# JuliaPhylo/PhyloGaussianBeliefProp.jl

Measured on AMD Instinct MI355X. Metric: clique-tree messages/sec (calibrate!: postorder+preorder), 16-trait BM, higher is better.
Workload: dtype f64; 1 GPU; cfg3: homogeneous BM, 16 traits, 50000-tip random bifurcating tree (seed 3), cliquetree, fixed root; clusters=99998, sepsets=99997, tree_depth=38, parallelism=single GPU

## Files before the change

### include/pgbp.h

```cpp
#ifndef PGBP_H
#define PGBP_H

#include <stdint.h>

#ifdef __cplusplus
extern "C" {
#endif

#define PGBP_VERSION 1
#define PGBP_MAX_DIM 384

enum pgbp_status {
  PGBP_OK = 0,
  PGBP_ERR_INVALID = 1,
  PGBP_ERR_HIP = 2,
  PGBP_ERR_NOT_TREE = 3,
  PGBP_ERR_TOO_LARGE = 4,
  PGBP_ERR_NO_DEVICE = 5,
  PGBP_ERR_STATE = 6
};

typedef struct pgbp_desc {
  int32_t n_clusters;
  int32_t n_sepsets;
// ... 35 lines not shown
                            const int32_t* pa_j, const int32_t* ch_j);
int64_t pgbp_plan_packed_size(const pgbp_plan* p);
int64_t pgbp_plan_residual_size(const pgbp_plan* p);
int32_t pgbp_plan_n_messages(const pgbp_plan* p);
int  pgbp_plan_traversal_sizes(const pgbp_plan* p, int32_t tree, int32_t dir,
                               int32_t* n_levels, int32_t* n_tasks, int32_t* n_entries);
int  pgbp_plan_traversal(const pgbp_plan* p, int32_t tree, int32_t dir, int32_t* level_off,
                         int32_t* task_off, int32_t* entry_msg, int32_t* entry_edge, int32_t* entry_reuse);
int  pgbp_plan_level_nfast(const pgbp_plan* p, int32_t tree, int32_t dir, int32_t* level_nfast);
int  pgbp_plan_groups(const pgbp_plan* p, int32_t tree, int32_t dir, int32_t* level_ngroups, int32_t* tail_levels,
                      int32_t* records, int32_t* tail_records);
int  pgbp_plan_chunks(const pgbp_plan* p, int32_t tree, int32_t dir, int32_t* n_chunks, int32_t* info, int32_t* wg_off,
                      int32_t* records);
int  pgbp_plan_prologues(const pgbp_plan* p, int32_t tree, int32_t dir, int32_t* level_pro, int32_t* tail_pro,
                         int32_t* chunk_pro);
int  pgbp_plan_chains(const pgbp_plan* p, int32_t tree, int32_t dir, int32_t* tail_chain, int32_t* chunk_chain);
int  pgbp_plan_records(const pgbp_plan* p, int32_t tree, int32_t dir, int32_t* n_records, int32_t* level_first,
                       int32_t* task_first, uint8_t* records);
int  pgbp_plan_rows(const pgbp_plan* p, int32_t tree, int32_t dir, int64_t* n_rows, int64_t* level_row0,
                    int32_t* level_nrows, int32_t* rowmap);
int  pgbp_plan_onschedule(const pgbp_plan* p, int32_t* n_levels, int32_t* cluster_level, int32_t* msg_level,
                          int32_t* walk_pos);
const char* pgbp_plan_last_error(const pgbp_plan* p);

int  pgbp_create(const pgbp_desc* desc, pgbp_engine** out);
void pgbp_destroy(pgbp_engine* e);
const char* pgbp_last_error(const pgbp_engine* e);
int64_t pgbp_packed_size(const pgbp_engine* e);
int64_t pgbp_residual_size(const pgbp_engine* e);
int32_t pgbp_n_messages(const pgbp_engine* e);
// ... 249 lines not shown
```

### phylogaussianbeliefprop.jl_amd/_lib.py

```python
import ctypes as C
import os

import numpy as np

os.environ.setdefault("HIP_FORCE_DEV_KERNARG", "1")

_HERE = os.path.dirname(os.path.abspath(__file__))
LIB_PATH = os.environ.get("PGBP_LIB", os.path.join(_HERE, "csrc", "libpgbp.so"))

PGBP_OK, ERR_INVALID, ERR_HIP, ERR_NOT_TREE, ERR_TOO_LARGE, ERR_NO_DEVICE, ERR_STATE = range(7)
PGBP_MAX_DIM = 384


class PgbpError(RuntimeError):
    def __init__(self, code, msg):
        super().__init__(f"pgbp error {code}: {msg}")
        self.code = code
        self.msg = msg


class Desc(C.Structure):
    _fields_ = [("n_clusters", C.c_int32), ("n_sepsets", C.c_int32),
                ("dims", C.POINTER(C.c_int32)), ("sepset_clusters", C.POINTER(C.c_int32)),
                ("scope_off", C.POINTER(C.c_int64)), ("scope_idx", C.POINTER(C.c_int32)),
# ... 38 lines not shown
_I64P = C.POINTER(C.c_int64)
_F64P = C.POINTER(C.c_double)
SYMBOLS = {
    "pgbp_plan_create": (C.c_int, [C.POINTER(Desc), C.POINTER(_P)]),
    "pgbp_plan_destroy": (None, [_P]),
    "pgbp_plan_set_schedule": (C.c_int, [_P, C.c_int32, _I32P, _I32P, _I32P]),
    "pgbp_plan_packed_size": (C.c_int64, [_P]),
    "pgbp_plan_residual_size": (C.c_int64, [_P]),
    "pgbp_plan_n_messages": (C.c_int32, [_P]),
    "pgbp_plan_traversal_sizes": (C.c_int, [_P, C.c_int32, C.c_int32, _I32P, _I32P, _I32P]),
    "pgbp_plan_traversal": (C.c_int, [_P, C.c_int32, C.c_int32, _I32P, _I32P, _I32P, _I32P, _I32P]),
    "pgbp_plan_level_nfast": (C.c_int, [_P, C.c_int32, C.c_int32, _I32P]),
    "pgbp_plan_groups": (C.c_int, [_P, C.c_int32, C.c_int32, _I32P, _I32P, _I32P, _I32P]),
    "pgbp_plan_chunks": (C.c_int, [_P, C.c_int32, C.c_int32, _I32P, _I32P, _I32P, _I32P]),
    "pgbp_plan_prologues": (C.c_int, [_P, C.c_int32, C.c_int32, _I32P, _I32P, _I32P]),
    "pgbp_plan_chains": (C.c_int, [_P, C.c_int32, C.c_int32, _I32P, _I32P]),
    "pgbp_plan_records": (C.c_int, [_P, C.c_int32, C.c_int32, _I32P, _I32P, _I32P, C.c_void_p]),
    "pgbp_plan_rows": (C.c_int, [_P, C.c_int32, C.c_int32, C.POINTER(C.c_int64), C.POINTER(C.c_int64), _I32P, _I32P]),
    "pgbp_plan_onschedule": (C.c_int, [_P, _I32P, _I32P, _I32P, _I32P]),
    "pgbp_residual_threshold": (C.c_double, [C.c_double, C.c_double]),
    "pgbp_plan_last_error": (C.c_char_p, [_P]),
    "pgbp_create": (C.c_int, [C.POINTER(Desc), C.POINTER(_P)]),
    "pgbp_destroy": (None, [_P]),
    "pgbp_last_error": (C.c_char_p, [_P]),
    "pgbp_packed_size": (C.c_int64, [_P]),
    "pgbp_residual_size": (C.c_int64, [_P]),
    "pgbp_n_messages": (C.c_int32, [_P]),
    "pgbp_belief_dim": (C.c_int32, [_P, C.c_int32]),
    "pgbp_set_beliefs": (C.c_int, [_P, _F64P, C.c_int32]),
    "pgbp_get_beliefs": (C.c_int, [_P, _F64P]),
# ... 192 lines not shown
```

### phylogaussianbeliefprop.jl_amd/csrc/pgbp_engine.hip

```cpp
#include <hip/hip_runtime.h>

#include <algorithm>
#include <climits>
#include <limits>
#include <cmath>
#include <cstdlib>
#include <cstdio>
#include <cstring>
#include <iterator>
#include <memory>
#include <string>
#include <vector>

#include "pgbp_devmem.hpp"
#include "pgbp_internal.hpp"
#include "pgbp_kernels.hpp"
#include "pgbp_lgmodel.hpp"
#include "pgbp_sites_host.hpp"
#include "pgbp_topology.hpp"

using namespace pgbp;

namespace {

// ... 209 lines not shown
  S.n_msgs = e->plan.n_msgs();
  S.update_resnorm = o ? o->update_residualnorm : 1;
  S.atol = o ? o->atol : 1e-5;
  S.thr = e->d_thr.get();
  S.logtab = reinterpret_cast<const double2*>(e->d_logtab.get());
  const int sp = e->plan.fast_p > 0 ? e->plan.fast_p : 0;
  S.thr_h_p = e->h_thr.empty() ? 0.0 : e->h_thr[sp];
  S.thr_J_p = e->h_thr.empty() ? 0.0 : e->h_thr[PGBP_MAX_DIM + 1 + sp];
  S.bs16 = e->layout_bs16 ? 1 : 0;
  S.fast_p = e->plan.fast_p;
  S.sm = e->layout_sm ? 1 : 0;
  S.n_sites = e->plan.n_sites;
  S.packed_off = e->d_packed_off.get();
  S.rpacked_off = e->d_rpacked_off.get();
  S.sep_zero = 0;
  S.notcal = nullptr;
  if (e->layout_sm) {
    S.pool = e->sm.pool.get();
    S.rpool = e->sm.rpool.get();
  }
  return S;
}

__global__ __launch_bounds__(256) void clear_poison_if_failed(const unsigned long long* __restrict__ fail, int n_sites,
                                                              int32_t* __restrict__ poison, int64_t n_words) {
  __shared__ int any;
  if (threadIdx.x == 0) any = 0;
  __syncthreads();
  for (int s = threadIdx.x; s < n_sites; s += blockDim.x)
    if (is_failure_key(fail[s])) any = 1;
// ... 205 lines not shown
      const int e0 = tr.task_off[t0], e1 = tr.task_off[t0 + nt];
      int level_s = 0;
      for (int q = e0; q < e1; ++q) level_s = std::max(level_s, (int)e->plan.msgs[tr.entries[q].msg].s);
      const auto b0 = std::lower_bound(d.kl_big.begin(), d.kl_big.end(), e0), b1 = std::lower_bound(d.kl_big.begin(), d.kl_big.end(), e1);
      const int n_big = (int)(b1 - b0);
      e->kl_flags_clean = e->kl_div_clean = false;
      if (n_big == 0 || ensure_ws(e, (int64_t)n_big * e->plan.n_sites * kldiv_ws_doubles(level_s)) == PGBP_OK)
        launch_residual_kldiv(S, d.d_entries.get(), e0, e1 - e0, level_s, e->d_kldiv.get(), e->d_klflags.get(), e->plan.n_sites, stop_below, e->st,
                              d.d_kl_big.get() + (b0 - d.kl_big.begin()), n_big, e->d_ws.get());
      else
        e->enqueue_rc = PGBP_ERR_HIP;
    }
  }
}

void enqueue_tree(pgbp_engine* e, const DevState& S, int tree, int dirs, unsigned long long pair_index, bool kl = false,
                  int* n_launches = nullptr) {
  const Tree& T = e->plan.trees[tree];
  const unsigned long long seq_base = pair_index * seq_stride(e);
  const unsigned long long stop_post = seq_base, stop_pre = seq_base + (unsigned long long)T.pa.size();
  const int np = (dirs & 1) ? tail_levels(e, T.post, kl) : 0, nq = (dirs & 2) ? tail_levels(e, T.pre, kl) : 0;
  const int nlev_post = (int)T.post.level_off.size() - 1, nlev_pre = (int)T.pre.level_off.size() - 1;
  if (dirs & 1) enqueue_levels(e, S, T.post, e->dpost[tree], 0, nlev_post - np, seq_base, stop_post, kl, n_launches);
  if (np + nq > 0) {
    const size_t first = (size_t)(np > 0 ? 0 : T.post.tail_levels) * kTailWaves;
    launch_loop_or_tail(e, S, e->d_tail[tree].get() + first, e->d_tail_pros[tree] ? e->d_tail_pros[tree].get() + first : nullptr, np + nq,
                        np, seq_base, stop_post, stop_pre, nullptr, 0);
    if (n_launches) *n_launches += 1;
  }
  if (dirs & 2) enqueue_levels(e, S, T.pre, e->dpre[tree], nq, nlev_pre, seq_base, stop_pre, kl, n_launches);
}

void enqueue_pair_and_iscal(pgbp_engine* e, const DevState& S, int tree, unsigned long long pair, bool kl, int32_t* d_out,
                            int* n_launches = nullptr) {
  const Plan& p = e->plan;
  const bool fused = e->layout_sm && !kl && S.update_resnorm != 0 && (int)p.trees[tree].pa.size() == p.n_sepsets;
  if (fused) {
    (void)hipMemsetAsync(e->d_notcal.get(), 0, sizeof(int32_t) * (size_t)p.n_sites, e->st);
    DevState S1 = S;
    S1.notcal = e->d_notcal.get();
    enqueue_tree(e, S1, tree, 3, pair, kl, n_launches);
    launch_iscal_from_notcal(e->d_notcal.get(), d_out, p.n_sites, e->st);
  } else {
    enqueue_tree(e, S, tree, 3, pair, kl, n_launches);
    launch_reduce_flags(e->d_flags.get(), p.n_msgs(), p.n_sites, d_out, e->st, e->layout_sm ? 1 : 0);
  }
}

void integrate_async(pgbp_engine* e, int belief, double* d_mu) {
  const Plan& p = e->plan;
  if (e->layout_sm)
    launch_integrate_sm(e->sm.pool.get(), p.packed_off[belief], p.dims[belief], d_mu, std::max(1, p.max_dim), e->d_norm.get(),
                        e->d_info.get(), p.n_sites, e->st);
  else if (ensure_ws(e, (int64_t)p.n_sites * big_ws_doubles(p.dims[belief])) == PGBP_OK)
    launch_integrate(e->d_pool.get(), p.pool_stride(), p.boff[belief], p.dims[belief], e->layout_bs16 ? 1 : 0, p.fast_p, d_mu,
                     std::max(1, p.max_dim), e->d_norm.get(), e->d_info.get(), p.n_sites, e->d_ws.get(), e->st);
  else
// ... 114 lines not shown
    {
      double tab[256];
      for (int i = 0; i < 128; ++i) {
        const long double c = 0.5L + ((long double)i + 0.5L) / 256.0L;
        const double inv = (double)(1.0L / c);
        tab[2 * i] = inv;
        tab[2 * i + 1] = (double)(-logl((long double)inv));
      }
      if (hipMemcpy(e->d_logtab.get(), tab, sizeof(tab), hipMemcpyHostToDevice) != hipSuccess) return bail(PGBP_ERR_HIP);
    }
  }
  if ((rc = dev_alloc(e, e->d_fail, ns))) return bail(rc);
  if ((rc = dev_alloc(e, e->d_poison, nsw * (size_t)p.n_clusters))) return bail(rc);
  if ((rc = dev_alloc(e, e->d_iscal, ns))) return bail(rc);
  if ((rc = dev_alloc(e, e->d_notcal, ns))) return bail(rc);
  if ((rc = upload(e, e->d_boff, p.boff))) return bail(rc);
  if ((rc = upload(e, e->d_packed_off, p.packed_off))) return bail(rc);
  if ((rc = upload(e, e->d_roff, p.roff))) return bail(rc);
  if ((rc = upload(e, e->d_rpacked_off, p.rpacked_off))) return bail(rc);
  if ((rc = dev_alloc(e, e->d_mu, ns * (size_t)std::max(1, p.max_dim)))) return bail(rc);
  if ((rc = dev_alloc(e, e->d_norm, ns))) return bail(rc);
  if ((rc = dev_alloc(e, e->d_info, ns))) return bail(rc);
  {
    std::vector<int32_t> rdim(nm);
    for (size_t d = 0; d < nm; ++d) rdim[d] = p.dims[p.n_clusters + d / 2];
    for (int32_t v : rdim) e->max_s = std::max(e->max_s, v);
    if ((rc = upload(e, e->d_bdim, p.dims))) return bail(rc);
    if ((rc = upload(e, e->d_rdim, rdim))) return bail(rc);
    if ((rc = dev_alloc(e, e->d_symflag, 1))) return bail(rc);
  }
// ... 1638 lines not shown
```

### phylogaussianbeliefprop.jl_amd/csrc/pgbp_fast.hip

```cpp
#include <hip/hip_runtime.h>

#include <algorithm>

#include "pgbp_bs16.hpp"
#include "pgbp_kernels.hpp"

#include "pgbp_fast_dev.hpp"

namespace pgbp {

constexpr int kSlotJ = 0, kSlotH = 256, kSlotG = 272, kSlotStatus = 273, kSlotDoubles = 288;

extern __shared__ double fast_lds[];

constexpr int kLevel = 0, kTail = 2;

#ifdef PGBP_STAMP
constexpr int kStampSlots = 1 << 16, kStampN = 12;
__device__ unsigned int g_stamp[kStampSlots][kStampN + 4];
__device__ unsigned int g_stamp_n;
#define PGBP_ST(i) do { stv[i] = (unsigned int)__builtin_amdgcn_s_memtime(); } while (0)
#else
#define PGBP_ST(i) do { } while (0)
#endif
// ... 69 lines not shown
      if (g == split && split > 0) {
        failkey = __hip_atomic_load(&S.fail[site], __ATOMIC_RELAXED, __HIP_MEMORY_SCOPE_AGENT);
        failkey = ((unsigned long long)(unsigned int)__builtin_amdgcn_readfirstlane((int)(failkey >> 32)) << 32) |
                  (unsigned long long)(unsigned int)__builtin_amdgcn_readfirstlane((int)(unsigned int)failkey);
      }
    }
    const unsigned long long stop_below = (MODE == kTail && g >= split) ? stop_b : stop_a;

    int state = (en.valid && !((failkey >> kInfoBits) < stop_below)) ? 1 : 0;
    const bool has_block = en.s > 0;
    const bool own = (en.mode & kFOwn) != 0;
    const bool accum = (en.mode & kFAccum) != 0;
    const bool recv_blk = has_block || (accum && !(en.mode & kFNoBlock));
    const bool provider = en.src_wave == wave;
    const int first_wave = en.grp_base;

    double* __restrict__ sep = pool + en.sep_off;
    double* __restrict__ to = pool + en.to_off;
    double* __restrict__ res = rpool + en.res_off;
    const int mt = en.mt, up0 = en.up0;
    const bool tpk = BS && (mt == P || mt == 2 * P);
    const int sepH = BS ? bs16::h1(P) : PR * PR, sepG = has_block ? (BS ? bs16::g1(P) : PR * PR + PR) : 0;
    const int64_t tJ0 = tpk ? ((mt == 2 * P && up0 == P) ? bs16::t11(P) : 0) : (up0 + (int64_t)mt * up0);
    const int64_t tH0 = (tpk ? (mt == P ? bs16::h1(P) : bs16::h2(P)) : (int64_t)mt * mt) + up0;
    const int64_t tG0 = tpk ? (mt == P ? bs16::g1(P) : bs16::g2(P)) : (int64_t)mt * mt + mt;

    Blk mJ{0, 0, 0, 0}, tJ{0, 0, 0, 0}, sJ{0, 0, 0, 0};
    double mh[2] = {0, 0}, gmsg = 0.0, th[2] = {0, 0}, tg = 0.0;
    double2 sh = make_double2(0.0, 0.0);
    double sg = 0.0;
    int info = 0;
    PGBP_ST(1);
    if (state == 1) {
      int zero_v = 0;
      if constexpr (MODE != kLevel) asm volatile("" : "+v"(zero_v));
      int poison_v = S.poison[(int64_t)site * S.n_clusters + en.from_b + zero_v];
      const bool pro = PRO && (en.mode & kFPro) != 0;
      if (pro) poison_v |= S.poison[(int64_t)site * S.n_clusters + pr.from_b + zero_v];
      auto load_sep_to = [&]() {
        if (!S.sep_zero) {
          if (has_block) {
            sJ = load_blk<BS, ODD, kStream, PL>(sep, PR, a, b, up, kidx, PR);
            if (b == 0) sh = load_pair<ODD>(sep + sepH, a, PR);
          }
          sg = sep[sepG];
        }
        if (own) {
          if (recv_blk) {
            tJ = load_blk<BS, ODD, false, PL>(to + tJ0, mt, a, b, up, kidx, PR);
            if (b == 0) {
              const double2 t2 = load_pair<ODD>(to + tH0, a, PR);
              th[0] = t2.x; th[1] = t2.y;
            }
          }
          tg = to[tG0];
// ... 118 lines not shown
              if (BS ? up : act) {
                maxJ2 = fmax(fmax(fabs(d2.x), fabs(d2.y)), fmax(fabs(d2.z), fabs(d2.w)));
                if (d2.x != d2.x || d2.y != d2.y || d2.z != d2.z || d2.w != d2.w) maxJ2 = INFINITY;
              }
              if (act && b == 0) {
                store_pair<ODD>(sep2 + xH, a, xh.x, xh.y, PR);
                store_pair<ODD, true>(res2 + xH, a, d2h0, d2h1, PR);
                maxh2 = (d2h0 != d2h0 || d2h1 != d2h1) ? INFINITY : fmax(fabs(d2h0), fabs(d2h1));
              }
              if (lane == 0) {
                sep2[xG] = xg;
                S.status[(int64_t)site * S.n_msgs + pr.msg] = 0;
              }
              if (S.update_resnorm) {
                const bool all_ok2 = __all(maxh2 <= S.thr_h_p && maxJ2 <= S.thr_J_p);
                if (lane == 0) S.flags[(int64_t)site * S.n_msgs + pr.msg] = all_ok2 ? 1 : 0;
              }
              f.w[0][0] += d2.x; f.w[1][0] += d2.y; f.w[0][1] += d2.z; f.w[1][1] += d2.w;
              f.h[0] += d2h0; f.h[1] += d2h1;
              gmsg += d2g;
              double* __restrict__ fw = pool + en.from_off;
              const int i0 = (en.keep0 == 0) ? PR : 0;
              double* __restrict__ iJ = BS ? fw + (en.keep0 == 0 ? bs16::t11(P) : 0) : fw + i0 + (int64_t)(2 * PR) * i0;
              double* __restrict__ iH = BS ? fw + bs16::h2(P) + (en.keep0 == 0 ? P : 0) : fw + 4 * PR * PR + i0;
              double* __restrict__ iG = BS ? fw + bs16::g2(P) : fw + 4 * PR * PR + 2 * PR;
              store_blk<BS, ODD, false, PL>(iJ, 2 * PR, a, b, up, act, kidx, Blk{f.w[0][0], f.w[1][0], f.w[0][1], f.w[1][1]}, PR);
              if (act && b == 0) store_pair<ODD>(iH, a, f.h[0], f.h[1], PR);
              if (lane == 0) iG[0] = gmsg;
            }
          }
          {
// ... 49 lines not shown
      const int pst = (int)src[kSlotStatus];
      if (pst == 1) {
        const double4 v = *reinterpret_cast<const double4*>(src + kSlotJ + 4 * lane);
        mJ = Blk{v.x, v.y, v.z, v.w};
        if (b == 0) {
          const double2 u = *reinterpret_cast<const double2*>(src + kSlotH + 2 * a);
          mh[0] = u.x; mh[1] = u.y;
        }
        gmsg = src[kSlotG];
      } else {
        state = 3;
      }
    }
    Blk dJ{0, 0, 0, 0};
    double dh0 = 0.0, dh1 = 0.0, dg = 0.0;
    if (state == 1) {
      double maxJ = 0.0, maxh = 0.0;
      if (has_block) {
        dJ = Blk{mJ.x - sJ.x, mJ.y - sJ.y, mJ.z - sJ.z, mJ.w - sJ.w};
        store_blk<BS, ODD, kStream, PL>(sep, PR, a, b, up, act, kidx, mJ, PR);
        store_blk<BS, ODD, true, PL>(res, PR, a, b, up, act, kidx, dJ, PR);
        if (BS ? up : act) {
          maxJ = fmax(fmax(fabs(dJ.x), fabs(dJ.y)), fmax(fabs(dJ.z), fabs(dJ.w)));
          if (dJ.x != dJ.x || dJ.y != dJ.y || dJ.z != dJ.z || dJ.w != dJ.w) maxJ = INFINITY;
        }
        if (act && b == 0) {
          dh0 = mh[0] - sh.x; dh1 = mh[1] - sh.y;
          store_pair<ODD, kStream>(sep + sepH, a, mh[0], mh[1], PR);
          store_pair<ODD, true>(res + (BS ? bs16::h1(P) : PR * PR), a, dh0, dh1, PR);
          maxh = (dh0 != dh0 || dh1 != dh1) ? INFINITY : fmax(fabs(dh0), fabs(dh1));
        }
      }
      dg = gmsg - sg;
      if (lane == 0) {
        sep[sepG] = gmsg;
        S.status[(int64_t)site * S.n_msgs + en.msg] = 0;
      }
      if (S.update_resnorm) {
        const bool lane_ok = maxh <= S.thr_h_p && maxJ <= S.thr_J_p;
        const bool all_ok = __all(lane_ok);
        if (lane == 0) S.flags[(int64_t)site * S.n_msgs + en.msg] = (!has_block || all_ok) ? 1 : 0;
      }
    } else if (state >= 2 && lane == 0) {
      S.poison[(int64_t)site * S.n_clusters + en.to_b] = 1;
      if (state == 2) {
        S.status[(int64_t)site * S.n_msgs + en.msg] = info;
        atomicMin(&S.fail[site], ((seq_base + (unsigned long long)en.seq) << kInfoBits) | (unsigned long long)info);
      }
    }
    if (accum && wave > first_wave) {
      if (state == 1) {
        *reinterpret_cast<double4*>(slot + kSlotJ + 4 * lane) = make_double4(dJ.x, dJ.y, dJ.z, dJ.w);
        if (act && b == 0) *reinterpret_cast<double2*>(slot + kSlotH + 2 * a) = make_double2(dh0, dh1);
      }
      if (lane == 0) {
        slot[kSlotG] = dg;
// ... 392 lines not shown
```

### phylogaussianbeliefprop.jl_amd/csrc/pgbp_internal.hpp

```cpp
#pragma once
#include <cstddef>
#include <cstdint>
#include <string>
#include <vector>

#include "../../include/pgbp.h"

namespace pgbp {

constexpr int kRecAlign = 16;
#if defined(__HIPCC__)
__host__ __device__
#endif
inline int64_t sm_row(int64_t n_sites) { return (n_sites + 31) / 32 * 32; }
constexpr int kWave = 64;

struct MsgDesc {
  int64_t from_off, to_off, sep_off, res_off;
  int32_t mf, mt, s, ni;
  int32_t keep_map, up_map, int_map;
  int32_t keep0;
  int32_t up0;
  int32_t from_b, to_b, sep_b;
};
static_assert(sizeof(MsgDesc) == 72 || sizeof(MsgDesc) == 80, "MsgDesc layout");

struct Entry {
  int32_t msg;
  int32_t edge;
  int32_t reuse;
  int32_t seq;
  int32_t tflags;
  int32_t pro;
  int32_t pad[2];
};
constexpr int kTLoad = 1, kTStore = 2;

struct URec {
  int32_t msg, seq, reuse, from_b, to_b;
  int32_t mf, s, mt, ni;
  int32_t k, i0, i1, u;
  int32_t pad[3];
  int64_t from_off, sep_off, to_off, res_off;
  int64_t from_p, sep_p, to_p, res_p;
};
static_assert(sizeof(URec) == 128, "URec layout");

constexpr int kGInlPerm = 40, kGInlUp = 16;
constexpr int kSmallI = 8, kSmallK = 8;
// ... 21 lines not shown
  uint8_t src_wave;
  uint8_t mode;
  uint8_t grp_base;
  uint8_t grp_len;
  uint8_t pad[6];
};
static_assert(sizeof(FEntry) == 64, "FEntry must be one 64-byte record");
void link_chains(std::vector<FEntry>& recs, const std::vector<struct FPro>& pros, const std::vector<std::pair<int64_t, int64_t>>& walks,
                 int P);
struct FPro {
  int64_t from_off, sep_off, res_off;
  int32_t msg, from_b;
};
static_assert(sizeof(FPro) == 32, "FPro is half a 64-byte line");
constexpr int kFOwn = 1, kFAccum = 2;
constexpr int kFPro = 8;
constexpr int kFNoBlock = 4;
constexpr int kFastMaxWaves = 4;
constexpr int kPassRotate = 3;
constexpr int kTailWaves = 8;
constexpr int kGenericMaxDim = 64;
inline bool big_msg(const MsgDesc& m) { return m.mf > kGenericMaxDim || m.mt > 254; }
constexpr int kLdsMaxDim = 128;
constexpr int kChunkMaxTasks = 2400;
constexpr int kChunkGenericMaxTasks = 4096;
constexpr int kChunkUniMaxThreads = 65536;
constexpr int kChunkGenericMaxMf = 24;
constexpr int kChunkDepth = 4;
constexpr int kChunkBins = 256;
constexpr int kChunkGenericDepth = 6;
constexpr int kSmall4MinTasksDefault = 1024;
constexpr size_t kMixedLevelFastMin = 2048;
constexpr size_t kMixedLevelFastMinNarrow = (size_t)1 << 30;

struct Tuning {
  bool tail = true;
  bool chunks = true;
  bool prologues = true;
  bool pair2 = true;
  bool loop2 = true;
  bool packed_layouts = true;
  long long mixed_fast_min = -1;
  int small4_min = kSmall4MinTasksDefault;
  int chunk_bins = -1;
};
bool read_tuning(Tuning& t, std::string& err);

struct Traversal {
  std::vector<int32_t> level_off;
  std::vector<int32_t> level_nfast;
  std::vector<int32_t> level_nbig;
  int32_t max_mf_big = 0;
  std::vector<FEntry> fentries;
  std::vector<FPro> fpros, tpros, cpros;
  bool has_pro = false;
  std::vector<int64_t> level_fbase;
  std::vector<int32_t> level_ngroups;
  std::vector<int32_t> level_nrecs;
// ... 95 lines not shown
```

### phylogaussianbeliefprop.jl_amd/csrc/pgbp_kernels.hip

```cpp
#include <hip/hip_runtime.h>

#include <algorithm>
#include <cstddef>
#include <cstdlib>

#include "pgbp_bs16.hpp"
#include "pgbp_kernels.hpp"
#include "pgbp_small_dev.hpp"

namespace pgbp {

#ifndef PGBP_SMALL_DPP
#define PGBP_SMALL_DPP 1
#endif
#ifndef PGBP_SMALL_SETTLE
#define PGBP_SMALL_SETTLE 1
#endif

static constexpr int kPermDoubles = PGBP_MAX_DIM / 2;

__device__ __forceinline__ double wave_max(double v) {
#pragma unroll
  for (int o = 32; o > 0; o >>= 1) v = fmax(v, __shfl_xor(v, o));
  return v;
// ... 2465 lines not shown
}

void launch_halt_if_calibrated(const int32_t* d_iscal, unsigned long long* d_fail, unsigned long long key, int n_sites,
                               hipStream_t st) {
  hipLaunchKernelGGL(halt_if_calibrated_kernel, dim3((n_sites + 63) / 64), dim3(64), 0, st, d_iscal, d_fail, key, n_sites);
}

__global__ void iscal_from_notcal_kernel(const int32_t* __restrict__ notcal, int32_t* __restrict__ iscal, int n_sites) {
  const int s = blockIdx.x * blockDim.x + threadIdx.x;
  if (s < n_sites) iscal[s] = notcal[s] == 0 ? 1 : 0;
}
void launch_iscal_from_notcal(const int32_t* d_notcal, int32_t* d_iscal, int n_sites, hipStream_t st) {
  hipLaunchKernelGGL(iscal_from_notcal_kernel, dim3((n_sites + 255) / 256), dim3(256), 0, st, d_notcal, d_iscal, n_sites);
}

void launch_reduce_flags(const int32_t* flags, int n_msgs, int n_sites, int32_t* d_iscal, hipStream_t st, int sm) {
  (void)hipMemsetAsync(d_iscal, 0x01, sizeof(int32_t) * (size_t)n_sites, st);
  if (n_msgs <= 0) return;
  if (sm) {
    const int bs = n_sites >= 256 ? 256 : 64;
    hipLaunchKernelGGL(reduce_flags_sm_kernel, dim3(n_msgs < 1024 ? n_msgs : 1024, (n_sites + bs - 1) / bs), dim3(bs), 0, st,
                       flags, n_msgs, n_sites, d_iscal);
    return;
  }
  hipLaunchKernelGGL(reduce_flags_kernel, dim3(grid_for(n_msgs, n_sites), n_sites), dim3(256), 0, st, flags,
                     n_msgs, d_iscal);
}

template <class T>
__global__ __launch_bounds__(256) void transpose_words_kernel(const T* __restrict__ src, T* __restrict__ dst, int n,
// ... 37 lines not shown
```

### phylogaussianbeliefprop.jl_amd/csrc/pgbp_kernels.hpp

```cpp
#pragma once
#include <hip/hip_runtime.h>

#include "pgbp_internal.hpp"
#include "pgbp_lgtable.hpp"

namespace pgbp {

constexpr unsigned long long kNoFail = ~0ull;
constexpr int kInfoBits = 20;

struct DevState {
  double* pool;
  int64_t pool_stride;
  double* rpool;
  int64_t rpool_stride;
  const MsgDesc* msgs;
  const int32_t* idx;
  int32_t* flags;
  int32_t* status;
  unsigned long long* fail;
  int32_t* poison;
  int32_t n_clusters;
  int32_t n_msgs;
  int32_t update_resnorm;
  double atol;
  const double* thr;
  double thr_h_p, thr_J_p;
  const double2* logtab;
  int32_t bs16;
  int32_t fast_p;
  int32_t sm;
  int32_t n_sites;
  const int64_t* packed_off;
  const int64_t* rpacked_off;
  int32_t* notcal;
  int32_t sep_zero;
};

size_t generic_lds_bytes(int max_mf);

#if defined(__HIPCC__)
__device__ __forceinline__ double log_by_table(const double2* __restrict__ tab, double x) {
  int e;
  const double m = frexp(x, &e);
  const int i = __builtin_amdgcn_readfirstlane((__double2hiint(m) >> 13) & 127);
  typedef double pgbp_cdouble2 __attribute__((ext_vector_type(2)));
  const __attribute__((address_space(4))) pgbp_cdouble2* ctab =
      reinterpret_cast<const __attribute__((address_space(4))) pgbp_cdouble2*>(reinterpret_cast<unsigned long long>(tab));
  const pgbp_cdouble2 tv = ctab[i];
  const double2 t = make_double2(tv.x, tv.y);
  const double r = fma(m, t.x, -1.0);
// ... 158 lines not shown
constexpr int kKlLdsMaxS = 96;
int64_t kldiv_ws_doubles(int s);
void launch_residual_kldiv(const DevState& S, const Entry* d_entries, int e0, int n_entries, int max_s, double* d_kldiv,
                           int32_t* d_klflags, int n_sites, unsigned long long stop_below, hipStream_t st,
                           const int32_t* d_big_ent = nullptr, int n_big = 0, double* d_ws = nullptr);

void launch_regularize_bycluster(double* pool, int64_t pool_stride, const int64_t* d_boff, const int32_t* d_dim,
                                 const int32_t* d_nb_off, const int32_t* d_nb_msg, const MsgDesc* d_msgs,
                                 const int32_t* d_idx, const int32_t* d_sepcl, double* d_eps, int n_clusters,
                                 int n_sepsets, int n_sites, hipStream_t st);
void launch_regularize_onschedule(double* pool, int64_t pool_stride, const int32_t* d_dim, const int32_t* d_a_cl, int a0,
                                  int n, const int32_t* d_ed_off, const int32_t* d_ed_msg, const MsgDesc* d_msgs,
                                  const int32_t* d_idx, int n_sites, hipStream_t st);
void launch_reduce_flags(const int32_t* flags, int n_msgs, int n_sites, int32_t* d_iscal, hipStream_t st, int sm = 0);
void launch_iscal_from_notcal(const int32_t* d_notcal, int32_t* d_iscal, int n_sites, hipStream_t st);
void launch_halt_if_calibrated(const int32_t* d_iscal, unsigned long long* d_fail, unsigned long long key, int n_sites,
                               hipStream_t st);
__host__ __device__ inline bool is_failure_key(unsigned long long key) { return key != kNoFail && (key & ((1ull << kInfoBits) - 1)) != 0; }

int engine_pack_gather_slot(pgbp_engine* e, int32_t slot_sites, double** d_slot, hipStream_t* st, int32_t* n_sites);
int engine_pack_records_device(pgbp_engine* e, int32_t site, int32_t n, const int32_t* beliefs, double* d_buf, int to_buf,
                               hipStream_t* st, int64_t* total);
int engine_fail(pgbp_engine* e, int code, const std::string& msg);
int engine_device(const pgbp_engine* e);
int engine_n_sites(const pgbp_engine* e);
struct EngineView {
  const Plan* plan;
  hipStream_t st;
  const double* pool;
  const int64_t* boff;
// ... 17 lines not shown
```

### phylogaussianbeliefprop.jl_amd/csrc/pgbp_loop.hip

```cpp
#include <hip/hip_runtime.h>

#include "pgbp_fast_dev.hpp"

namespace pgbp {

extern __shared__ double loop_lds[];

#ifdef PGBP_STAMP
constexpr int kLStampSlots = 1 << 16, kLStampN = 12;
__device__ unsigned int g_lstamp[kLStampSlots][kLStampN + 4];
__device__ unsigned int g_lstamp_n;
#define PGBP_LT(i) do { stv[i] = (unsigned int)__builtin_amdgcn_s_memtime(); } while (0)
#else
#define PGBP_LT(i) do { } while (0)
#endif

namespace {

constexpr int kLSlotJ = 0, kLSlotH = 256, kLSlotG = 272, kLSlotStatus = 273, kLSlotInfo = 274, kLSlotDoubles = 288;
constexpr int kLoopWaves = 2 * kTailWaves;

struct SndOps {
  Blk ii, ss;
  double2 t0, t1;
// ... 338 lines not shown
      [[maybe_unused]] const bool pro = PRO && (en.mode & kFPro) != 0;
      const int chain_kind = first_pass ? 0 : en.pad[0], chain_src = en.pad[1];
      FEntry nx{};
      FPro npr{};

      double* __restrict__ sep = pool + en.sep_off;
      double* __restrict__ to = pool + en.to_off;
      double* __restrict__ res = rpool + en.res_off;
      const int mt = en.mt, up0 = en.up0;
      const bool tpk = (mt == P || mt == 2 * P);
      const int sepG = has_block ? bs16::g1(P) : 0;
      const int64_t tJ0 = tpk ? ((mt == 2 * P && up0 == P) ? bs16::t11(P) : 0) : (up0 + (int64_t)mt * up0);
      const int64_t tH0 = (tpk ? (mt == P ? bs16::h1(P) : bs16::h2(P)) : (int64_t)mt * mt) + up0;
      const int64_t tG0 = tpk ? (mt == P ? bs16::g1(P) : bs16::g2(P)) : (int64_t)mt * mt + mt;
      const bool sepz = S.sep_zero != 0;
      issue_next();
      const int f_ii = en.keep0 == 0 ? bs16::t11(P) : 0, f_hi = bs16::h2(P) + (en.keep0 == 0 ? P : 0);
      Blk sJ{0, 0, 0, 0}, tJ{0, 0, 0, 0};
      double2 sh = make_double2(0.0, 0.0);
      double sg = 0.0, th0 = 0.0, th1 = 0.0, tg = 0.0;
      Blk p_x{0, 0, 0, 0}, p_d{0, 0, 0, 0}, p_ii{0, 0, 0, 0};
      double p_xh0 = 0.0, p_xh1 = 0.0, p_dh0 = 0.0, p_dh1 = 0.0, p_xg = 0.0, p_h0 = 0.0, p_h1 = 0.0, p_g = 0.0;
      bool p_ok = false;
      if (live) {
        if (!sepz) {
          if (has_block) {
            sJ = load_blk<true, false, !PRO, PL>(sep, P, a, b, up, kidx);
            if (b == 0) sh = load_pair<false>(sep + bs16::h1(P), a, P);
          }
          sg = sep[sepG];
        }
        if (own) {
          if (recv_blk) {
            tJ = load_blk<true, false, false, PL>(to + tJ0, mt, a, b, up, kidx);
            if (b == 0) {
              const double2 t2 = load_pair<false>(to + tH0, a, P);
              th0 = t2.x; th1 = t2.y;
            }
          }
          tg = to[tG0];
// ... 30 lines not shown
          p_xh0 = xh.x; p_xh1 = xh.y;
          p_d = Blk{p_x.x - s2.x, p_x.y - s2.y, p_x.z - s2.z, p_x.w - s2.w};
          p_dh0 = xh.x - s2h.x; p_dh1 = xh.y - s2h.y;
          const double d2g = p_xg - s2g;
          p_ii = Blk{fi.x + p_d.x, fi.y + p_d.y, fi.z + p_d.z, fi.w + p_d.w};
          p_h0 = fh.x + p_dh0; p_h1 = fh.y + p_dh1;
          p_g = fg + d2g;
        }
      }
      if (accum && wave > first_wave && live) {
        *reinterpret_cast<double4*>(delta + kLSlotJ + 4 * lane) = make_double4(sJ.x, sJ.y, sJ.z, sJ.w);
        if (act && b == 0) *reinterpret_cast<double2*>(delta + kLSlotH + 2 * a) = sh;
        if (lane == 0) delta[kLSlotG] = sg;
      }
      asm volatile("s_waitcnt vmcnt(0)" ::: "memory");
      PGBP_LT(4);
      lds_barrier();
      PGBP_LT(5);
      Blk mJ{0, 0, 0, 0};
      double mh0 = 0.0, mh1 = 0.0, gmsg = 0.0;
      int state = 0, info = 0;
      if (live) {
        const double* src = loop_lds + en.src_wave * kLSlotDoubles;
        state = (int)src[kLSlotStatus];
        info = (int)src[kLSlotInfo];
        if (state == 1) {
          const double4 v = *reinterpret_cast<const double4*>(src + kLSlotJ + 4 * lane);
          mJ = Blk{v.x, v.y, v.z, v.w};
          if (b == 0) {
            const double2 u = *reinterpret_cast<const double2*>(src + kLSlotH + 2 * a);
// ... 68 lines not shown
        if (up) {
          maxJ2 = fmax(fmax(fabs(p_d.x), fabs(p_d.y)), fmax(fabs(p_d.z), fabs(p_d.w)));
          if (p_d.x != p_d.x || p_d.y != p_d.y || p_d.z != p_d.z || p_d.w != p_d.w) maxJ2 = INFINITY;
        }
        if (act && b == 0) {
          store_pair<false>(sep2 + xH, a, p_xh0, p_xh1, P);
          store_pair<false, true>(res2 + xH, a, p_dh0, p_dh1, P);
          maxh2 = (p_dh0 != p_dh0 || p_dh1 != p_dh1) ? INFINITY : fmax(fabs(p_dh0), fabs(p_dh1));
        }
        if (lane == 0) {
          sep2[xG] = p_xg;
          S.status[(int64_t)site * S.n_msgs + pr.msg] = 0;
        }
        if (S.update_resnorm) {
          const bool all_ok2 = __all(maxh2 <= S.thr_h_p && maxJ2 <= S.thr_J_p);
          if (lane == 0) S.flags[(int64_t)site * S.n_msgs + pr.msg] = all_ok2 ? 1 : 0;
        }
        store_blk<true, false, false, PL>(fw + f_ii, P, a, b, up, act, kidx, p_ii);
        if (act && b == 0) store_pair<false>(fw + f_hi, a, p_h0, p_h1, P);
        if (lane == 0) fw[bs16::g2(P)] = p_g;
      }
      if (state == 1) {
        if (has_block) {
          store_blk<true, false, !PRO, PL>(sep, P, a, b, up, act, kidx, mJ);
          store_blk<true, false, true, PL>(res, P, a, b, up, act, kidx, dJ);
          if (act && b == 0) {
            store_pair<false, !PRO>(sep + bs16::h1(P), a, mh0, mh1, P);
            store_pair<false, true>(res + bs16::h1(P), a, dh0, dh1, P);
          }
        }
        if (lane == 0) {
          sep[sepG] = gmsg;
          S.status[(int64_t)site * S.n_msgs + en.msg] = 0;
        }
        if (S.update_resnorm) {
          const bool lane_ok = maxh <= S.thr_h_p && maxJ <= S.thr_J_p;
          const bool all_ok = __all(lane_ok);
          if (lane == 0) S.flags[(int64_t)site * S.n_msgs + en.msg] = (!has_block || all_ok) ? 1 : 0;
        }
        if (own) {
          if (recv_blk) {
            store_blk<true, false, false, PL>(to + tJ0, mt, a, b, up, act, kidx, tJ);
            if (act && b == 0) store_pair<false>(to + tH0, a, th0, th1, P);
          }
          if (lane == 0) to[tG0] = tg;
        }
      } else if (state >= 2 && lane == 0) {
        S.poison[(int64_t)site * S.n_clusters + en.to_b] = 1;
        if (state == 2) {
          S.status[(int64_t)site * S.n_msgs + en.msg] = info;
          atomicMin(&S.fail[site], ((seq_base + (unsigned long long)en.seq) << kInfoBits) | (unsigned long long)info);
        }
      }
// ... 77 lines not shown
```

### phylogaussianbeliefprop.jl_amd/csrc/pgbp_plan.cpp

```cpp
#include <algorithm>
#include <array>
#include <cerrno>
#include <climits>
#include <cstdlib>
#include <cstring>
#include <map>
#include <set>
#include <unordered_map>

#include "pgbp_internal.hpp"

namespace pgbp {

static int64_t pad_to(int64_t n, int64_t a) { return (n + a - 1) / a * a; }

bool read_tuning(Tuning& t, std::string& err) {
  t = Tuning{};
  const char* v = getenv("PGBP_TUNING");
  if (!v) return true;
  std::string all(v);
  size_t at = 0;
  while (at <= all.size()) {
    size_t end = all.find(',', at);
    if (end == std::string::npos) end = all.size();
// ... 9 lines not shown
    bool numeric = false;
    if (!flag) {
      char* stop = nullptr;
      errno = 0;
      num = strtoll(tok.c_str() + eq + 1, &stop, 10);
      numeric = stop != tok.c_str() + eq + 1 && *stop == '\0' && errno == 0;
    }
    auto within = [&](long long lo, long long hi) { return numeric && num >= lo && num <= hi; };
    bool ok = false;
    if (key == "no_tail") { ok = flag; t.tail = false; }
    else if (key == "no_chunks") { ok = flag; t.chunks = false; }
    else if (key == "no_prologue") { ok = flag; t.prologues = false; }
    else if (key == "plain_layout") { ok = flag; t.packed_layouts = false; }
    else if (key == "pair") { ok = within(0, 1); t.pair2 = num != 0; }
    else if (key == "loop") { ok = within(0, 1); t.loop2 = num != 0; }
    else if (key == "mixed_fast_min") { ok = within(-1, LLONG_MAX); t.mixed_fast_min = num; }
    else if (key == "small4_min") { ok = within(-1, INT_MAX); t.small4_min = (int)num; }
    else if (key == "chunk_bins") { ok = within(0, INT_MAX); t.chunk_bins = (int)num; }
    if (!ok) {
      err = "PGBP_TUNING: unknown key or bad value in token '" + tok + "'";
      return false;
    }
  }
  return true;
}

int plan_build(Plan& p, const pgbp_desc* d) {
  if (!d || d->n_clusters <= 0 || d->n_sepsets < 0 || !d->dims || d->n_sites < 1) {
    p.err = "invalid description (null pointers, no clusters, or n_sites < 1)";
    return PGBP_ERR_INVALID;
// ... 196 lines not shown
      f.keep0 = (uint8_t)(m.keep0 < 0 ? 0 : m.keep0);
      f.up0 = (uint8_t)(m.s > 0 ? m.up0 : 0);
      if (!en.reuse) provider = fill + w;
      f.src_wave = (uint8_t)provider;
      f.grp_base = (uint8_t)fill;
      f.grp_len = (uint8_t)len;
      if (accum) {
        f.mode = (uint8_t)(kFAccum | (w == 0 ? kFOwn : 0) | (blk.second < 0 ? kFNoBlock : 0));
        if (w == 0 && m.s == 0) {
          f.up0 = (uint8_t)blk.first;
          f.mt = (uint8_t)(blk.second >= 0 ? blk.second : m.mt);
        }
      } else {
        f.mode = kFOwn;
      }
      if (pending) {
        const MsgDesc& x = p.msgs[pending->msg];
        f.mode |= kFPro;
        fp.from_off = x.from_off; fp.sep_off = x.sep_off; fp.res_off = x.res_off;
        fp.msg = pending->msg; fp.from_b = x.from_b;
        pending = nullptr;
        if (any_pro) *any_pro = true;
      }
      out.push_back(f);
      out_pro.push_back(fp);
      ++w;
    }
    fill += len;
  }
  for (; fill < W; ++fill) {
// ... 654 lines not shown
          Entry e{};
          e.msg = msg_to(i, t.ch[i]);
          e.edge = i;
          e.seq = n + i;
          e.reuse = 0;
          e.pro = 1;
          tr.entries.push_back(e);
          tr.max_mf = std::max(tr.max_mf, p.msgs[e.msg].mf);
        }
        for (int i : tk) {
          Entry e{};
          e.msg = msg_to(i, t.ch[i]);
          e.edge = i;
          e.seq = n + i;
          e.reuse = 0;
          if (prev_msg >= 0) {
            const MsgDesc& a = p.msgs[prev_msg];
            const MsgDesc& b = p.msgs[e.msg];
            if (a.from_b == b.from_b && a.s == b.s && b.ni > 0 &&
                std::equal(p.idxpool.begin() + a.keep_map, p.idxpool.begin() + a.keep_map + a.s,
                           p.idxpool.begin() + b.keep_map))
              e.reuse = 1;
          }
          prev_msg = e.msg;
          tr.entries.push_back(e);
          tr.max_mf = std::max(tr.max_mf, p.msgs[e.msg].mf);
        }
        tr.task_off.push_back((int)tr.entries.size());
      }
      if (!tasks.empty()) tr.level_off.push_back((int)tr.task_off.size() - 1);
// ... 365 lines not shown
  if (tail_pro) dump(tr->tentries, tr->tpros, 0, tr->tentries.size(), tail_pro);
  if (chunk_pro) {
    size_t o = 0;
    for (const auto& ch : tr->chunks) {
      const size_t nrec = (size_t)ch.n_groups * pgbp::kTailWaves;
      if (ch.generic)
        std::fill(chunk_pro + o, chunk_pro + o + nrec, -1);
      else
        dump(tr->centries, tr->cpros, (size_t)ch.group0 * pgbp::kTailWaves, (size_t)ch.group0 * pgbp::kTailWaves + nrec, chunk_pro + o);
      o += nrec;
    }
  }
  return PGBP_OK;
}

int pgbp_plan_chains(const pgbp_plan* p, int32_t tree, int32_t dir, int32_t* tail_chain, int32_t* chunk_chain) {
  const pgbp::Traversal* tr = get_trav(p, tree, dir);
  if (!tr) return PGBP_ERR_INVALID;
  auto word = [](const pgbp::FEntry& f) { return (int32_t)f.pad[0] | ((int32_t)f.pad[1] << 8) | ((int32_t)f.pad[2] << 16); };
  if (tail_chain) {
    const pgbp::Tree& T = p->p.trees[tree];
    const size_t first = dir == 0 ? 0 : T.post.tentries.size();
    for (size_t i = 0; i < tr->tentries.size(); ++i) tail_chain[i] = word(T.tail[first + i]);
  }
  if (chunk_chain) {
    size_t o = 0;
    for (const auto& ch : tr->chunks) {
      const size_t nrec = (size_t)ch.n_groups * pgbp::kTailWaves;
      for (size_t i = 0; i < nrec; ++i)
        chunk_chain[o + i] = ch.generic ? 0 : word(tr->centries[(size_t)ch.group0 * pgbp::kTailWaves + i]);
// ... 43 lines not shown
```

Measured before the change: 259.8 million messages/s.

## Skip sepset loads for leaf preorder messages and fuse calibration check

In the preorder pass, messages to leaf clusters whose upward message fully covered the sepset are marked in the plan. For these the kernel takes the sepset from the just-computed target values instead of loading it from memory. Residual failures are also recorded per site in a notcal array, and a new kernel combines that array with a flag scan, done only when the fail key shows one is needed, replacing the full flag reduction. This cuts global memory reads for about half the messages and the per-call flag reduction, at the cost of added plan metadata and a correctness dependency on the leaf-sepset equality assumption.

```diff
diff --git a/include/pgbp.h b/include/pgbp.h
--- a/include/pgbp.h
+++ b/include/pgbp.h
@@ -73,6 +73,8 @@
                       int32_t* records);
 int  pgbp_plan_prologues(const pgbp_plan* p, int32_t tree, int32_t dir, int32_t* level_pro, int32_t* tail_pro,
                          int32_t* chunk_pro);
+int  pgbp_plan_leaf_sepset(const pgbp_plan* p, int32_t tree, int32_t dir, int32_t* level_leaf, int32_t* tail_leaf,
+                           int32_t* chunk_leaf);
 int  pgbp_plan_chains(const pgbp_plan* p, int32_t tree, int32_t dir, int32_t* tail_chain, int32_t* chunk_chain);
 int  pgbp_plan_records(const pgbp_plan* p, int32_t tree, int32_t dir, int32_t* n_records, int32_t* level_first,
                        int32_t* task_first, uint8_t* records);
diff --git a/phylogaussianbeliefprop.jl_amd/_lib.py b/phylogaussianbeliefprop.jl_amd/_lib.py
--- a/phylogaussianbeliefprop.jl_amd/_lib.py
+++ b/phylogaussianbeliefprop.jl_amd/_lib.py
@@ -76,6 +76,7 @@
     "pgbp_plan_groups": (C.c_int, [_P, C.c_int32, C.c_int32, _I32P, _I32P, _I32P, _I32P]),
     "pgbp_plan_chunks": (C.c_int, [_P, C.c_int32, C.c_int32, _I32P, _I32P, _I32P, _I32P]),
     "pgbp_plan_prologues": (C.c_int, [_P, C.c_int32, C.c_int32, _I32P, _I32P, _I32P]),
+    "pgbp_plan_leaf_sepset": (C.c_int, [_P, C.c_int32, C.c_int32, _I32P, _I32P, _I32P]),
     "pgbp_plan_chains": (C.c_int, [_P, C.c_int32, C.c_int32, _I32P, _I32P]),
     "pgbp_plan_records": (C.c_int, [_P, C.c_int32, C.c_int32, _I32P, _I32P, _I32P, C.c_void_p]),
     "pgbp_plan_rows": (C.c_int, [_P, C.c_int32, C.c_int32, C.POINTER(C.c_int64), C.POINTER(C.c_int64), _I32P, _I32P]),
diff --git a/phylogaussianbeliefprop.jl_amd/csrc/pgbp_engine.hip b/phylogaussianbeliefprop.jl_amd/csrc/pgbp_engine.hip
--- a/phylogaussianbeliefprop.jl_amd/csrc/pgbp_engine.hip
+++ b/phylogaussianbeliefprop.jl_amd/csrc/pgbp_engine.hip
@@ -247,6 +247,7 @@
   S.packed_off = e->d_packed_off.get();
   S.rpacked_off = e->d_rpacked_off.get();
   S.sep_zero = 0;
+  S.leaf_sepset = 0;
   S.notcal = nullptr;
   if (e->layout_sm) {
     S.pool = e->sm.pool.get();
@@ -482,11 +483,13 @@
   }
 }
 
-void enqueue_tree(pgbp_engine* e, const DevState& S, int tree, int dirs, unsigned long long pair_index, bool kl = false,
+void enqueue_tree(pgbp_engine* e, const DevState& S_in, int tree, int dirs, unsigned long long pair_index, bool kl = false,
                   int* n_launches = nullptr) {
   const Tree& T = e->plan.trees[tree];
   const unsigned long long seq_base = pair_index * seq_stride(e);
   const unsigned long long stop_post = seq_base, stop_pre = seq_base + (unsigned long long)T.pa.size();
+  DevState S = S_in;
+  S.leaf_sepset = (dirs == 3 && !kl && e->plan.tune.leaf_sepset && e->plan.all_fast && !uni_engine(e) && !e->layout_sm) ? 1 : 0;
   const int np = (dirs & 1) ? tail_levels(e, T.post, kl) : 0, nq = (dirs & 2) ? tail_levels(e, T.pre, kl) : 0;
   const int nlev_post = (int)T.post.level_off.size() - 1, nlev_pre = (int)T.pre.level_off.size() - 1;
   if (dirs & 1) enqueue_levels(e, S, T.post, e->dpost[tree], 0, nlev_post - np, seq_base, stop_post, kl, n_launches);
@@ -503,12 +506,20 @@
                             int* n_launches = nullptr) {
   const Plan& p = e->plan;
   const bool fused = e->layout_sm && !kl && S.update_resnorm != 0 && (int)p.trees[tree].pa.size() == p.n_sepsets;
+  const bool fused_fast = !fused && leaf_mark_grid(p.fast_p + (p.fast_p & 1)) && !e->layout_sm && !uni_engine(e) && p.all_fast && !kl && S.update_resnorm != 0 &&
+                          (int)p.trees[tree].pa.size() == p.n_sepsets && !p.trees[tree].post.has_pro && !p.trees[tree].pre.has_pro;
   if (fused) {
     (void)hipMemsetAsync(e->d_notcal.get(), 0, sizeof(int32_t) * (size_t)p.n_sites, e->st);
     DevState S1 = S;
     S1.notcal = e->d_notcal.get();
     enqueue_tree(e, S1, tree, 3, pair, kl, n_launches);
     launch_iscal_from_notcal(e->d_notcal.get(), d_out, p.n_sites, e->st);
+  } else if (fused_fast) {
+    DevState S1 = S;
+    S1.notcal = e->d_notcal.get();
+    enqueue_tree(e, S1, tree, 3, pair, kl, n_launches);
+    launch_iscal_from_notcal_or_flags(e->d_notcal.get(), e->d_flags.get(), p.n_msgs(), e->d_fail.get(), (pair + 1) * seq_stride(e), d_out,
+                                      p.n_sites, e->st);
   } else {
     enqueue_tree(e, S, tree, 3, pair, kl, n_launches);
     launch_reduce_flags(e->d_flags.get(), p.n_msgs(), p.n_sites, d_out, e->st, e->layout_sm ? 1 : 0);
@@ -653,6 +664,7 @@
   if ((rc = dev_alloc(e, e->d_poison, nsw * (size_t)p.n_clusters))) return bail(rc);
   if ((rc = dev_alloc(e, e->d_iscal, ns))) return bail(rc);
   if ((rc = dev_alloc(e, e->d_notcal, ns))) return bail(rc);
+  if (hipMemsetAsync(e->d_notcal.get(), 0, sizeof(int32_t) * ns, e->st) != hipSuccess) return bail(PGBP_ERR_HIP);
   if ((rc = upload(e, e->d_boff, p.boff))) return bail(rc);
   if ((rc = upload(e, e->d_packed_off, p.packed_off))) return bail(rc);
   if ((rc = upload(e, e->d_roff, p.roff))) return bail(rc);
diff --git a/phylogaussianbeliefprop.jl_amd/csrc/pgbp_fast.hip b/phylogaussianbeliefprop.jl_amd/csrc/pgbp_fast.hip
--- a/phylogaussianbeliefprop.jl_amd/csrc/pgbp_fast.hip
+++ b/phylogaussianbeliefprop.jl_amd/csrc/pgbp_fast.hip
@@ -107,6 +107,7 @@
     const bool recv_blk = has_block || (accum && !(en.mode & kFNoBlock));
     const bool provider = en.src_wave == wave;
     const int first_wave = en.grp_base;
+    const bool leafsep = leaf_mark_grid(P) && en.pad[3] != 0 && S.leaf_sepset != 0;
 
     double* __restrict__ sep = pool + en.sep_off;
     double* __restrict__ to = pool + en.to_off;
@@ -131,7 +132,7 @@
       const bool pro = PRO && (en.mode & kFPro) != 0;
       if (pro) poison_v |= S.poison[(int64_t)site * S.n_clusters + pr.from_b + zero_v];
       auto load_sep_to = [&]() {
-        if (!S.sep_zero) {
+        if (!S.sep_zero && !leafsep) {
           if (has_block) {
             sJ = load_blk<BS, ODD, kStream, PL>(sep, PR, a, b, up, kidx, PR);
             if (b == 0) sh = load_pair<ODD>(sep + sepH, a, PR);
@@ -280,7 +281,12 @@
               }
               if (S.update_resnorm) {
                 const bool all_ok2 = __all(maxh2 <= S.thr_h_p && maxJ2 <= S.thr_J_p);
-                if (lane == 0) S.flags[(int64_t)site * S.n_msgs + pr.msg] = all_ok2 ? 1 : 0;
+                if (lane == 0) {
+                  S.flags[(int64_t)site * S.n_msgs + pr.msg] = all_ok2 ? 1 : 0;
+                  if constexpr (leaf_mark_grid(P)) {
+                    if (!all_ok2 && S.notcal) S.notcal[site] = 1;
+                  }
+                }
               }
               f.w[0][0] += d2.x; f.w[1][0] += d2.y; f.w[0][1] += d2.z; f.w[1][1] += d2.w;
               f.h[0] += d2h0; f.h[1] += d2h1;
@@ -360,6 +366,11 @@
     }
     Blk dJ{0, 0, 0, 0};
     double dh0 = 0.0, dh1 = 0.0, dg = 0.0;
+    if (leafsep) {
+      sJ = tJ;
+      sh = make_double2(th[0], th[1]);
+      sg = tg;
+    }
     if (state == 1) {
       double maxJ = 0.0, maxh = 0.0;
       if (has_block) {
@@ -385,7 +396,12 @@
       if (S.update_resnorm) {
         const bool lane_ok = maxh <= S.thr_h_p && maxJ <= S.thr_J_p;
         const bool all_ok = __all(lane_ok);
-        if (lane == 0) S.flags[(int64_t)site * S.n_msgs + en.msg] = (!has_block || all_ok) ? 1 : 0;
+        if (lane == 0) {
+          S.flags[(int64_t)site * S.n_msgs + en.msg] = (!has_block || all_ok) ? 1 : 0;
+          if constexpr (leaf_mark_grid(P)) {
+            if (has_block && !all_ok && S.notcal) S.notcal[site] = 1;
+          }
+        }
       }
     } else if (state >= 2 && lane == 0) {
       S.poison[(int64_t)site * S.n_clusters + en.to_b] = 1;
diff --git a/phylogaussianbeliefprop.jl_amd/csrc/pgbp_internal.hpp b/phylogaussianbeliefprop.jl_amd/csrc/pgbp_internal.hpp
--- a/phylogaussianbeliefprop.jl_amd/csrc/pgbp_internal.hpp
+++ b/phylogaussianbeliefprop.jl_amd/csrc/pgbp_internal.hpp
@@ -32,7 +32,8 @@
   int32_t seq;
   int32_t tflags;
   int32_t pro;
-  int32_t pad[2];
+  int32_t leafsep;
+  int32_t pad[1];
 };
 constexpr int kTLoad = 1, kTStore = 2;
 
@@ -84,6 +85,7 @@
 };
 static_assert(sizeof(FPro) == 32, "FPro is half a 64-byte line");
 constexpr int kFOwn = 1, kFAccum = 2;
+constexpr bool leaf_mark_grid(int P) { return P != 2 && P != 10 && P != 14; }
 constexpr int kFPro = 8;
 constexpr int kFNoBlock = 4;
 constexpr int kFastMaxWaves = 4;
@@ -112,6 +114,7 @@
   bool packed_layouts = true;
   long long mixed_fast_min = -1;
   int small4_min = kSmall4MinTasksDefault;
+  bool leaf_sepset = true;
   int chunk_bins = -1;
 };
 bool read_tuning(Tuning& t, std::string& err);
diff --git a/phylogaussianbeliefprop.jl_amd/csrc/pgbp_kernels.hip b/phylogaussianbeliefprop.jl_amd/csrc/pgbp_kernels.hip
--- a/phylogaussianbeliefprop.jl_amd/csrc/pgbp_kernels.hip
+++ b/phylogaussianbeliefprop.jl_amd/csrc/pgbp_kernels.hip
@@ -2503,6 +2503,25 @@
   hipLaunchKernelGGL(iscal_from_notcal_kernel, dim3((n_sites + 255) / 256), dim3(256), 0, st, d_notcal, d_iscal, n_sites);
 }
 
+__global__ __launch_bounds__(256) void iscal_from_notcal_or_flags_kernel(int32_t* __restrict__ notcal, const int32_t* __restrict__ flags,
+                                                                         int n_msgs, const unsigned long long* __restrict__ fail,
+                                                                         unsigned long long seq_end, int32_t* __restrict__ iscal) {
+  const int site = blockIdx.x;
+  int bad = notcal[site] != 0;
+  if ((fail[site] >> kInfoBits) < seq_end)
+    for (int d = threadIdx.x; d < n_msgs; d += blockDim.x) bad |= (flags[(int64_t)site * n_msgs + d] == 0);
+  bad = __syncthreads_or(bad);
+  if (threadIdx.x == 0) {
+    iscal[site] = bad ? 0 : 1;
+    notcal[site] = 0;
+  }
+}
+void launch_iscal_from_notcal_or_flags(int32_t* d_notcal, const int32_t* d_flags, int n_msgs, const unsigned long long* d_fail,
+                                       unsigned long long seq_end, int32_t* d_iscal, int n_sites, hipStream_t st) {
+  hipLaunchKernelGGL(iscal_from_notcal_or_flags_kernel, dim3(n_sites), dim3(256), 0, st, d_notcal, d_flags, n_msgs, d_fail, seq_end,
+                     d_iscal);
+}
+
 void launch_reduce_flags(const int32_t* flags, int n_msgs, int n_sites, int32_t* d_iscal, hipStream_t st, int sm) {
   (void)hipMemsetAsync(d_iscal, 0x01, sizeof(int32_t) * (size_t)n_sites, st);
   if (n_msgs <= 0) return;
diff --git a/phylogaussianbeliefprop.jl_amd/csrc/pgbp_kernels.hpp b/phylogaussianbeliefprop.jl_amd/csrc/pgbp_kernels.hpp
--- a/phylogaussianbeliefprop.jl_amd/csrc/pgbp_kernels.hpp
+++ b/phylogaussianbeliefprop.jl_amd/csrc/pgbp_kernels.hpp
@@ -35,6 +35,7 @@
   const int64_t* rpacked_off;
   int32_t* notcal;
   int32_t sep_zero;
+  int32_t leaf_sepset;
 };
 
 size_t generic_lds_bytes(int max_mf);
@@ -223,6 +224,8 @@
                                   const int32_t* d_idx, int n_sites, hipStream_t st);
 void launch_reduce_flags(const int32_t* flags, int n_msgs, int n_sites, int32_t* d_iscal, hipStream_t st, int sm = 0);
 void launch_iscal_from_notcal(const int32_t* d_notcal, int32_t* d_iscal, int n_sites, hipStream_t st);
+void launch_iscal_from_notcal_or_flags(int32_t* d_notcal, const int32_t* d_flags, int n_msgs, const unsigned long long* d_fail,
+                                       unsigned long long seq_end, int32_t* d_iscal, int n_sites, hipStream_t st);
 void launch_halt_if_calibrated(const int32_t* d_iscal, unsigned long long* d_fail, unsigned long long key, int n_sites,
                                hipStream_t st);
 __host__ __device__ inline bool is_failure_key(unsigned long long key) { return key != kNoFail && (key & ((1ull << kInfoBits) - 1)) != 0; }
diff --git a/phylogaussianbeliefprop.jl_amd/csrc/pgbp_loop.hip b/phylogaussianbeliefprop.jl_amd/csrc/pgbp_loop.hip
--- a/phylogaussianbeliefprop.jl_amd/csrc/pgbp_loop.hip
+++ b/phylogaussianbeliefprop.jl_amd/csrc/pgbp_loop.hip
@@ -376,6 +376,7 @@
       const int64_t tH0 = (tpk ? (mt == P ? bs16::h1(P) : bs16::h2(P)) : (int64_t)mt * mt) + up0;
       const int64_t tG0 = tpk ? (mt == P ? bs16::g1(P) : bs16::g2(P)) : (int64_t)mt * mt + mt;
       const bool sepz = S.sep_zero != 0;
+      const bool leafsep = !PRO && leaf_mark_grid(P) && en.pad[3] != 0 && S.leaf_sepset != 0;
       issue_next();
       const int f_ii = en.keep0 == 0 ? bs16::t11(P) : 0, f_hi = bs16::h2(P) + (en.keep0 == 0 ? P : 0);
       Blk sJ{0, 0, 0, 0}, tJ{0, 0, 0, 0};
@@ -385,7 +386,7 @@
       double p_xh0 = 0.0, p_xh1 = 0.0, p_dh0 = 0.0, p_dh1 = 0.0, p_xg = 0.0, p_h0 = 0.0, p_h1 = 0.0, p_g = 0.0;
       bool p_ok = false;
       if (live) {
-        if (!sepz) {
+        if (!sepz && !leafsep) {
           if (has_block) {
             sJ = load_blk<true, false, !PRO, PL>(sep, P, a, b, up, kidx);
             if (b == 0) sh = load_pair<false>(sep + bs16::h1(P), a, P);
@@ -446,6 +447,11 @@
         if (lane == 0) delta[kLSlotG] = sg;
       }
       asm volatile("s_waitcnt vmcnt(0)" ::: "memory");
+      if (leafsep) {
+        sJ = tJ;
+        sh = make_double2(th0, th1);
+        sg = tg;
+      }
       PGBP_LT(4);
       lds_barrier();
       PGBP_LT(5);
@@ -544,7 +550,9 @@
         }
         if (S.update_resnorm) {
           const bool all_ok2 = __all(maxh2 <= S.thr_h_p && maxJ2 <= S.thr_J_p);
-          if (lane == 0) S.flags[(int64_t)site * S.n_msgs + pr.msg] = all_ok2 ? 1 : 0;
+          if (lane == 0) {
+            S.flags[(int64_t)site * S.n_msgs + pr.msg] = all_ok2 ? 1 : 0;
+          }
         }
         store_blk<true, false, false, PL>(fw + f_ii, P, a, b, up, act, kidx, p_ii);
         if (act && b == 0) store_pair<false>(fw + f_hi, a, p_h0, p_h1, P);
@@ -566,7 +574,12 @@
         if (S.update_resnorm) {
           const bool lane_ok = maxh <= S.thr_h_p && maxJ <= S.thr_J_p;
           const bool all_ok = __all(lane_ok);
-          if (lane == 0) S.flags[(int64_t)site * S.n_msgs + en.msg] = (!has_block || all_ok) ? 1 : 0;
+          if (lane == 0) {
+            S.flags[(int64_t)site * S.n_msgs + en.msg] = (!has_block || all_ok) ? 1 : 0;
+            if constexpr (!PRO && leaf_mark_grid(P)) {
+              if (has_block && !all_ok && S.notcal) S.notcal[site] = 1;
+            }
+          }
         }
         if (own) {
           if (recv_blk) {
diff --git a/phylogaussianbeliefprop.jl_amd/csrc/pgbp_plan.cpp b/phylogaussianbeliefprop.jl_amd/csrc/pgbp_plan.cpp
--- a/phylogaussianbeliefprop.jl_amd/csrc/pgbp_plan.cpp
+++ b/phylogaussianbeliefprop.jl_amd/csrc/pgbp_plan.cpp
@@ -47,6 +47,7 @@
     else if (key == "plain_layout") { ok = flag; t.packed_layouts = false; }
     else if (key == "pair") { ok = within(0, 1); t.pair2 = num != 0; }
     else if (key == "loop") { ok = within(0, 1); t.loop2 = num != 0; }
+    else if (key == "leaf_sepset") { ok = within(0, 1); t.leaf_sepset = num != 0; }
     else if (key == "mixed_fast_min") { ok = within(-1, LLONG_MAX); t.mixed_fast_min = num; }
     else if (key == "small4_min") { ok = within(-1, INT_MAX); t.small4_min = (int)num; }
     else if (key == "chunk_bins") { ok = within(0, INT_MAX); t.chunk_bins = (int)num; }
@@ -273,6 +274,7 @@
       } else {
         f.mode = kFOwn;
       }
+      if (!postorder && en.leafsep) f.pad[3] = 1;
       if (pending) {
         const MsgDesc& x = p.msgs[pending->msg];
         f.mode |= kFPro;
@@ -957,6 +959,10 @@
           e.edge = i;
           e.seq = n + i;
           e.reuse = 0;
+          {
+            const MsgDesc& up = p.msgs[msg_to(i, t.pa[i])];
+            e.leafsep = (!nchild.count(t.ch[i]) && up.ni == 0 && up.s == up.mf) ? 1 : 0;
+          }
           if (prev_msg >= 0) {
             const MsgDesc& a = p.msgs[prev_msg];
             const MsgDesc& b = p.msgs[e.msg];
@@ -1352,6 +1358,29 @@
   return PGBP_OK;
 }
 
+int pgbp_plan_leaf_sepset(const pgbp_plan* p, int32_t tree, int32_t dir, int32_t* level_leaf, int32_t* tail_leaf,
+                          int32_t* chunk_leaf) {
+  const pgbp::Traversal* tr = get_trav(p, tree, dir);
+  if (!tr) return PGBP_ERR_INVALID;
+  auto dump = [](const std::vector<pgbp::FEntry>& v, size_t i0, size_t i1, int32_t* out) {
+    for (size_t i = i0; i < i1; ++i) out[i - i0] = v[i].pad[3];
+  };
+  if (level_leaf) dump(tr->fentries, 0, tr->fentries.size(), level_leaf);
+  if (tail_leaf) dump(tr->tentries, 0, tr->tentries.size(), tail_leaf);
+  if (chunk_leaf) {
+    size_t o = 0;
+    for (const auto& ch : tr->chunks) {
+      const size_t nrec = (size_t)ch.n_groups * pgbp::kTailWaves;
+      if (ch.generic)
+        std::fill(chunk_leaf + o, chunk_leaf + o + nrec, 0);
+      else
+        dump(tr->centries, (size_t)ch.group0 * pgbp::kTailWaves, (size_t)ch.group0 * pgbp::kTailWaves + nrec, chunk_leaf + o);
+      o += nrec;
+    }
+  }
+  return PGBP_OK;
+}
+
 int pgbp_plan_chains(const pgbp_plan* p, int32_t tree, int32_t dir, int32_t* tail_chain, int32_t* chunk_chain) {
   const pgbp::Traversal* tr = get_trav(p, tree, dir);
   if (!tr) return PGBP_ERR_INVALID;
```

After: 263.6 million messages/s (median of 6 runs). 1.4% higher.
